# andreeaiana/manner

Hardware: AMD Instinct MI355X
Metric: candidate news encoded+scored/sec (higher is better)
Workload: dtype f16; 1 GPU; configs[1]: CR-Module late fusion, MIND-small shape (65238-news pool), bert-base-uncased architectu~; modules=1, parallelism=dp1 (impressions sharded, no collective)

## Files before the change

manner_amd/csrc/gemm.hip:

```cpp
#include <stdlib.h>

#include <type_traits>

#include "train_common.h"
#include "gemm_w4_asm.inc"
#include "gemm_w8_asm.inc"
#ifdef MANNER_P4_LAB
#include "gemm_p4_asm.inc"
#endif

namespace manner {
namespace {

constexpr int BM = 128, BN = 128, ROW_BYTES = 128, TILE_BYTES = 128 * ROW_BYTES;
constexpr int STAGE_BYTES = 2 * TILE_BYTES;

__device__ __forceinline__ float gelu_erf(float x) {
  return 0.5f * x * (1.0f + erff(x * 0.70710678118654752440f));
}

__device__ __forceinline__ float gelu_erf_fast(float x) {
  const float z = fabsf(x) * 0.70710678118654752440f;
  const float t = __builtin_amdgcn_rcpf(fmaf(0.3275911f, z, 1.0f));
  float p = fmaf(1.061405429f, t, -1.453152027f);
// ... 766 lines not shown
    } else {
      f32x4 bv[4], g4[4];
#pragma unroll
      for (int a = 0; a < 4; ++a) {
        bv[a] = *reinterpret_cast<const f32x4*>(bias + nbase + 16 * a + 4 * lq);
        g4[a] = *reinterpret_cast<const f32x4*>(dln.vec + nbase + 16 * a + 4 * lq);
      }
      char* rslab0 = slab;
      const int rrow0 = el >> 3, rsl = el & 7;
#pragma unroll
      for (int hb = 0; hb < (MBT + 3) / 4; ++hb) {
        const int nsb = MBT / 2 - 2 * hb >= 2 ? 2 : 1;
        const int nb4 = 2 * nsb;
        f32x4 rawres[2][4];
        float2 ms[4];
#pragma unroll
        for (int sb = 0; sb < nsb; ++sb)
#pragma unroll
          for (int q = 0; q < 4; ++q) {
            const int row = 8 * q + rrow0;
            const int m = min(mrow0 + 64 * hb + 32 * sb + row, M - 1);
            rawres[sb][q] = ABL == 3 ? f32x4{0.f, 0.f, 0.f, 0.f} : *reinterpret_cast<const f32x4*>(R + (size_t)m * N + nbase + 8 * (rsl ^ (row & 7)));
          }
#pragma unroll
        for (int b4 = 0; b4 < nb4; ++b4) ms[b4] = dln.mr[min(mrow0 + 16 * (4 * hb + b4) + l15, M - 1)];
        e16x4 res[4][4];
        if constexpr (!ONE_SLAB) {
#pragma unroll
          for (int sb = 0; sb < nsb; ++sb)
#pragma unroll
            for (int q = 0; q < 4; ++q) {
              const int row = 8 * q + rrow0;
              *reinterpret_cast<f32x4*>((sb ? rslab1 : rslab0) + row * 128 + (rsl << 4)) = rawres[sb][q];
            }
          __builtin_amdgcn_wave_barrier();
#pragma unroll
          for (int b4 = 0; b4 < nb4; ++b4) {
            const int row = 16 * (b4 & 1) + l15;
            const char* rs_ = (b4 >> 1) ? rslab1 : rslab0;
#pragma unroll
            for (int a = 0; a < 4; ++a) {
              const int c = (16 * a + 4 * lq) / 8;
              res[b4][a] = *reinterpret_cast<const e16x4*>(rs_ + row * 128 + ((c ^ (row & 7)) << 4) + 8 * (lq & 1));
            }
          }
          __builtin_amdgcn_wave_barrier();
        } else {
#pragma unroll
          for (int sb = 0; sb < nsb; ++sb) {
#pragma unroll
            for (int q = 0; q < 4; ++q) {
              const int row = 8 * q + rrow0;
              *reinterpret_cast<f32x4*>(rslab0 + row * 128 + (rsl << 4)) = rawres[sb][q];
            }
            __builtin_amdgcn_wave_barrier();
#pragma unroll
            for (int b2 = 0; b2 < 2; ++b2) {
              const int row = 16 * b2 + l15;
#pragma unroll
              for (int a = 0; a < 4; ++a) {
                const int c = (16 * a + 4 * lq) / 8;
                res[2 * sb + b2][a] = *reinterpret_cast<const e16x4*>(rslab0 + row * 128 + ((c ^ (row & 7)) << 4) + 8 * (lq & 1));
              }
            }
            __builtin_amdgcn_wave_barrier();
          }
        }
#pragma unroll
        for (int b4 = 0; b4 < nb4; ++b4) {
          const int bb = 4 * hb + b4;
          const float rs = ms[b4].y, nm = -ms[b4].x * ms[b4].y;
          float p1 = 0.f, p2 = 0.f;
#pragma unroll
          for (int a = 0; a < 4; ++a)
#pragma unroll
            for (int e = 0; e < 4; ++e) {
              const float r = fmaf((float)res[b4][a][e], rs, nm);
              const float x = fmaf(r, g4[a][e], acc[a][bb][e] + bv[a][e]);
              acc[a][bb][e] = x;
              p1 += x;
              p2 = fmaf(x, x, p2);
            }
          p1 += __shfl_xor(p1, 16, 64); p2 += __shfl_xor(p2, 16, 64);
          p1 += __shfl_xor(p1, 32, 64); p2 += __shfl_xor(p2, 32, 64);
          const int m = mrow0 + 16 * bb + l15;
          if (ABL == 4) asm volatile("" ::"v"(p1), "v"(p2));
          else if (ABL != 2 && lq == 0 && m < M)
            __hip_atomic_store(reinterpret_cast<unsigned long long*>(&dln.part[(size_t)(4 * nt + wn) * dln.part_stride + m]),
                               __builtin_bit_cast(unsigned long long, float2{p1, p2}), __ATOMIC_RELAXED, __HIP_MEMORY_SCOPE_AGENT);
        }
      }
    }
    if (ABL != 1) {
      const int row0 = el >> 3, sl = el & 7;
#pragma unroll
      for (int j = 0; j < MBT / 2; ++j) {
#pragma unroll
        for (int b2 = 0; b2 < 2; ++b2) {
          const int row = 16 * b2 + l15;
#pragma unroll
          for (int a = 0; a < 4; ++a) {
            const int c = (16 * a + 4 * lq) / 8;
            store4<TE>(reinterpret_cast<TE*>(slab + row * 128 + ((c ^ (row & 7)) << 4) + 8 * (lq & 1)),
                           acc[a][2 * j + b2][0], acc[a][2 * j + b2][1], acc[a][2 * j + b2][2], acc[a][2 * j + b2][3]);
          }
        }
        __builtin_amdgcn_wave_barrier();
#pragma unroll
        for (int q = 0; q < 4; ++q) {
          const int row = 8 * q + row0;
          const int c = sl ^ (row & 7);
          const int m = mrow0 + 32 * j + row;
          const f32x4 raw = *reinterpret_cast<const f32x4*>(slab + row * 128 + (sl << 4));
          if (m < M) *reinterpret_cast<f32x4*>(reinterpret_cast<TE*>(Y) + (size_t)m * N + nbase + 8 * c) = raw;
        }
        __builtin_amdgcn_wave_barrier();
      }
    }
    return;
  }
  int el = lane;
  asm volatile("" : "+v"(el));
  const int l15 = el & 15, lq = el >> 4, wn = ew & 3, wm = ew >> 2;
  const int nbase = nt * G_BN + wn * 64;
  const int row0 = el / CHUNKS, sl = el % CHUNKS;
  f32x4 bv[4];
#pragma unroll
  for (int a = 0; a < 4; ++a) bv[a] = *reinterpret_cast<const f32x4*>(bias + nbase + 16 * a + 4 * lq);
  constexpr bool NORM = EPI == EPI_NORM || EPI == EPI_NORM_GELU;
  constexpr bool SPLIT = EPI == EPI_BIAS_GELU_SPLIT3;
  const size_t ldy = SPLIT ? (size_t)3 * N : (size_t)N;
  f32x4 cv[NORM ? 4 : 1];
  float2 ms[NORM ? MBT : 1];
  const int mrow0 = mt * TM + wm * WROWS;
  if constexpr (NORM) {
#pragma unroll
    for (int a = 0; a < 4; ++a) cv[a] = *reinterpret_cast<const f32x4*>(dln.vec + nbase + 16 * a + 4 * lq);
#pragma unroll
    for (int bb = 0; bb < MBT; ++bb) ms[bb] = dln.mr[min(mrow0 + 16 * bb + l15, M - 1)];
  }
  constexpr int SLAB_ROWS = 4096 / OUT_ROW;
  constexpr int MB = SLAB_ROWS / 16;
  constexpr int SQ = SLAB_ROWS / ROWS_PER_INST;
#pragma unroll
  for (int j = 0; j < WROWS / SLAB_ROWS; ++j) {
#pragma unroll
    for (int b2 = 0; b2 < MB; ++b2) {
      const int row = 16 * b2 + l15;
#pragma unroll
      for (int a = 0; a < 4; ++a) {
        const int nl = 16 * a + 4 * lq;
        float v[4];
#pragma unroll
        for (int e = 0; e < 4; ++e) {
          if constexpr (NORM) v[e] = fmaf(ms[MB * j + b2].y, fmaf(-ms[MB * j + b2].x, cv[a][e], acc[a][MB * j + b2][e]), bv[a][e]);
          else v[e] = acc[a][MB * j + b2][e] + bv[a][e];
        }
        if (EPI == EPI_BIAS_GELU || EPI == EPI_NORM_GELU || SPLIT) {
#pragma unroll
          for (int e = 0; e < 4; ++e) v[e] = SPLIT ? gelu_erf_fast(v[e]) : sizeof(TOut) == 4 ? gelu_erf(v[e]) : gelu_poly(v[e]);
        }
        const int c = nl / OPC;
        const int off = row * OUT_ROW + ((c ^ (row & (CHUNKS - 1))) << 4) + (sizeof(TOut) == 2 ? 8 * (lq & 1) : 0);
        if constexpr (SPLIT) {
          typedef TOut o4 __attribute__((ext_vector_type(4)));
          o4 hv;
#pragma unroll
          for (int e = 0; e < 4; ++e) hv[e] = (TOut)v[e];
          asm volatile("" : "+v"(hv));
          *reinterpret_cast<o4*>(slab + off) = hv;
#pragma unroll
          for (int e = 0; e < 4; ++e) acc[a][MB * j + b2][e] = v[e] - (float)hv[e];
        } else {
          store4<TOut>(reinterpret_cast<TOut*>(slab + off), v[0], v[1], v[2], v[3]);
        }
      }
    }
    __builtin_amdgcn_wave_barrier();
    if constexpr (SPLIT) {
#pragma unroll
      for (int q = 0; q < SQ; ++q) {
        const int row = q * ROWS_PER_INST + row0;
        const int c = sl ^ (row & (CHUNKS - 1));
        const int m = mrow0 + SLAB_ROWS * j + row;
        const f32x4 raw = *reinterpret_cast<const f32x4*>(slab + row * OUT_ROW + (sl << 4));
        if (m < M) {
          TOut* dst = Y + (size_t)m * ldy + nbase + c * OPC;
          __builtin_nontemporal_store(raw, reinterpret_cast<f32x4*>(dst));
          __builtin_nontemporal_store(raw, reinterpret_cast<f32x4*>(dst + N));
        }
      }
      __builtin_amdgcn_wave_barrier();
#pragma unroll
      for (int b2 = 0; b2 < MB; ++b2) {
        const int row = 16 * b2 + l15;
#pragma unroll
        for (int a = 0; a < 4; ++a) {
          const int c = (16 * a + 4 * lq) / OPC;
          const int off = row * OUT_ROW + ((c ^ (row & (CHUNKS - 1))) << 4) + 8 * (lq & 1);
          store4<TOut>(reinterpret_cast<TOut*>(slab + off), acc[a][MB * j + b2][0], acc[a][MB * j + b2][1], acc[a][MB * j + b2][2],
                       acc[a][MB * j + b2][3]);
        }
      }
      __builtin_amdgcn_wave_barrier();
#pragma unroll
      for (int q = 0; q < SQ; ++q) {
        const int row = q * ROWS_PER_INST + row0;
        const int c = sl ^ (row & (CHUNKS - 1));
        const int m = mrow0 + SLAB_ROWS * j + row;
        const f32x4 raw = *reinterpret_cast<const f32x4*>(slab + row * OUT_ROW + (sl << 4));
        if (m < M) __builtin_nontemporal_store(raw, reinterpret_cast<f32x4*>(Y + (size_t)m * ldy + 2 * (size_t)N + nbase + c * OPC));
      }
      __builtin_amdgcn_wave_barrier();
      continue;
    }
    e16x4 res[EPI == EPI_BIAS_RES ? SQ : 1];
    f32x4 resf[EPI == EPI_BIAS_RES_F32 ? SQ : 1];
    if ((EPI == EPI_BIAS_RES || EPI == EPI_BIAS_RES_F32) && ABL != 1) {
#pragma unroll
      for (int q = 0; q < SQ; ++q) {
        const int row = q * ROWS_PER_INST + row0;
        const int m = min(mrow0 + SLAB_ROWS * j + row, M - 1);
        const size_t idx = (size_t)m * N + nbase + (sl ^ (row & (CHUNKS - 1))) * OPC;
        if (EPI == EPI_BIAS_RES) res[q] = *reinterpret_cast<const e16x4*>(R + idx);
        else resf[q] = *reinterpret_cast<const f32x4*>(reinterpret_cast<const float*>(R) + idx);
      }
    }
    f32x4 pre16v[EPI == EPI_GELU_GRAD16 ? SQ : 1];
    if constexpr (EPI == EPI_GELU_GRAD16) {
#pragma unroll
      for (int q = 0; q < SQ; ++q) {
        const int row = q * ROWS_PER_INST + row0;
        const int m = min(mrow0 + SLAB_ROWS * j + row, M - 1);
        pre16v[q] = *reinterpret_cast<const f32x4*>(static_cast<const TE*>(dln.pre16) + (size_t)m * N + nbase + (sl ^ (row & (CHUNKS - 1))) * OPC);
      }
    }
    f32x4 pre[EPI == EPI_GELU_GRAD ? SQ : 1][2];
    if constexpr (EPI == EPI_GELU_GRAD) {
#pragma unroll
      for (int q = 0; q < SQ; ++q) {
        const int row = q * ROWS_PER_INST + row0;
        const int m = min(mrow0 + SLAB_ROWS * j + row, M - 1);
        const f32x4* ip = reinterpret_cast<const f32x4*>(dln.aux32 + (size_t)m * N + nbase + (sl ^ (row & (CHUNKS - 1))) * OPC);
        pre[q][0] = ip[0];
        pre[q][1] = ip[1];
      }
    }
#pragma unroll
    for (int q = 0; q < SQ; ++q) {
      const int row = q * ROWS_PER_INST + row0;
      const int c = sl ^ (row & (CHUNKS - 1));
      const int m = mrow0 + SLAB_ROWS * j + row;
      f32x4 raw = *reinterpret_cast<const f32x4*>(slab + row * OUT_ROW + (sl << 4));
      if (ABL == 1) { asm volatile("" ::"v"(raw)); continue; }
      if constexpr (EPI == EPI_GELU_GRAD) {
        e16x8 d = __builtin_bit_cast(e16x8, raw);
#pragma unroll
        for (int e = 0; e < 8; ++e) d[e] = (TE)((float)d[e] * gelu_grad_fast(pre[q][e >> 2][e & 3]));
        raw = __builtin_bit_cast(f32x4, d);
      }
      if constexpr (EPI == EPI_GELU_GRAD16) {
        e16x8 d = __builtin_bit_cast(e16x8, raw);
        const e16x8 pv = __builtin_bit_cast(e16x8, pre16v[q]);
#pragma unroll
        for (int e = 0; e < 8; ++e) d[e] = (TE)((float)d[e] * gelu_grad_fast((float)pv[e]));
        raw = __builtin_bit_cast(f32x4, d);
      }
      if (EPI == EPI_BIAS_RES) {
#pragma unroll
        for (int e = 0; e < 4; ++e) raw[e] += (float)res[q][e];
      }
      if (EPI == EPI_BIAS_RES_F32) {
        if (dln.drop_thr != 0) {
          const uint64_t di = (uint64_t)(dln.drop_rowmap ? dln.drop_rowmap[min(m, M - 1)] : m) * N + (nbase + c * OPC);
#pragma unroll
          for (int e = 0; e < 4; ++e) raw[e] = drop_bits(dln.drop_seed, dln.drop_site, di + e) >= dln.drop_thr ? raw[e] * dln.drop_scale : 0.f;
        }
        raw += resf[q];
      }
      if (m < M) {
        f32x4* dst = reinterpret_cast<f32x4*>(reinterpret_cast<char*>(Y) + ((size_t)m * N + nbase + c * OPC) * sizeof(TOut));
        if (NORM && ABL != 5 && !dln.plain_stores) __builtin_nontemporal_store(raw, dst);
        else *dst = raw;
        if constexpr (EPI == EPI_BIAS_GELU_DUAL) {
          e16x4 gv;
#pragma unroll
          for (int e = 0; e < 4; ++e) gv[e] = (TE)gelu_erf_fast(raw[e]);
          *reinterpret_cast<e16x4*>(static_cast<TE*>(dln.aux16) + (size_t)m * N + nbase + c * OPC) = gv;
        }
        if constexpr (EPI == EPI_BIAS_GELU_DUAL16) {
          const e16x8 pv = __builtin_bit_cast(e16x8, raw);
          e16x8 gv;
#pragma unroll
          for (int e = 0; e < 8; ++e) gv[e] = (TE)gelu_erf_fast((float)pv[e]);
          *reinterpret_cast<e16x8*>(static_cast<TE*>(dln.aux16) + (size_t)m * N + nbase + c * OPC) = gv;
        }
      }
    }
    __builtin_amdgcn_wave_barrier();
  }
}


template <int TM>
__device__ __forceinline__ void nres_fan_in(const DlnAux& dln, int mt, int M, int n_tiles, int wave, int lane) {
  asm volatile("s_waitcnt vmcnt(0)" ::: "memory");
  __syncthreads();
  if (wave != 0) return;
  int old = 0;
  if (lane == 0) old = __hip_atomic_fetch_add(dln.fin_arrive + mt, 1, __ATOMIC_RELAXED, __HIP_MEMORY_SCOPE_AGENT);
  old = __builtin_amdgcn_readfirstlane(old);
  if (old != n_tiles - 1) return;
  constexpr int RPL = TM / 64;
  float2 v[RPL][16];
#pragma unroll
  for (int q = 0; q < RPL; ++q) {
    const int m = min(mt * TM + 64 * q + lane, M - 1);
#pragma unroll
    for (int g = 0; g < 16; ++g)
      v[q][g] = g < dln.fin_groups ? __builtin_bit_cast(float2, __hip_atomic_load(reinterpret_cast<const unsigned long long*>(&dln.part[(size_t)g * dln.part_stride + m]),
                                                                                  __ATOMIC_RELAXED, __HIP_MEMORY_SCOPE_AGENT))
                                   : float2{0.f, 0.f};
  }
#pragma unroll
  for (int q = 0; q < RPL; ++q) {
    const int m = mt * TM + 64 * q + lane;
    if (m < M) dln.fin_mr[m] = dln_row_stats(v[q], dln.fin_inv_h, dln.fin_eps);
  }
  if (lane == 0) __hip_atomic_store(dln.fin_arrive + mt, 0, __ATOMIC_RELAXED, __HIP_MEMORY_SCOPE_AGENT);
}

template <typename TE, typename TOut, int EPI, int ABL, int MBT>
__device__ __forceinline__ void gemm_tn_x16_body(
    char* lds, const TE* __restrict__ X, const TE* __restrict__ W, const float* __restrict__ bias,
    const TE* __restrict__ R, TOut* __restrict__ Y, int N, int K, int M, int n_tiles, const DlnAux& dln) {
  typedef TE TIn;
  typedef typename E16<TE>::v8 e16x8;
  constexpr int EPC = 8, BK = 64;
  constexpr int TM = 32 * MBT;
  constexpr int HB = MBT / 2;
  constexpr int WROWS = TM / 2;
  static_assert(MBT == 8 || MBT == 6, "row panels of 256 or 192 rows");
  constexpr int XB = 2 * G_OP_BYTES;

  const int G = gridDim.x, b = blockIdx.x;
  const int m_tiles = (MBT == 8 && dln.split_cus > 0) ? split_panels((M + TM - 1) / TM, n_tiles, dln.split_cus) : (M + TM - 1) / TM;
  const int valid_tiles = m_tiles * n_tiles;
  const int gsz = dln.col_group > 0 && dln.col_group < n_tiles ? dln.col_group : n_tiles;
  const int per_group = m_tiles * gsz;
  auto decode = [&](int tile, int& mt_, int& nt_) {
    const int g = tile / per_group;
    const int r = tile - g * per_group;
    const int width = min(gsz, n_tiles - g * gsz);
    mt_ = r / width;
    nt_ = g * gsz + (r - mt_ * width);
  };
  const TileWalk walk = tile_walk(G, b, valid_tiles, dln.xcd_ranges);
  int t = walk.first;
  if (t >= walk.end) return;
  if (dln.stagger > 0) {
    const int phase = (walk.first / n_tiles) & 3;
    for (int i = 0; i < phase * dln.stagger; ++i) __builtin_amdgcn_s_sleep(64);
  }

  const int tid = threadIdx.x, wave = __builtin_amdgcn_readfirstlane(tid >> 6), lane = tid & 63;
  const int kl15 = lane & 15, klq = lane >> 4;
  const int kwn = wave & 3, kwm = wave >> 2;

  const bool is_w = wave < 4;
  const int prow0 = is_w ? 64 * (wave & 3) : (TM / 4) * (wave & 3);
  const int ldst0 = (is_w ? 0 : XB) + prow0 * ROW_BYTES;
  const int lrow = lane >> 3;
  int voff[2];
#pragma unroll
  for (int par = 0; par < 2; ++par)
    voff[par] = lrow * K + (((lane & 7) ^ ((4 * par + (lane >> 4)) & 7)) * EPC);
  struct Src { const TIn* p; int lim; };
  auto tile_src = [&](int tile) -> Src {
    int mt_, nt_;
    decode(tile, mt_, nt_);
    if (is_w) return Src{W + (size_t)(nt_ * G_BN + prow0) * K, 64};
    if constexpr (MBT == 8) {
      return Src{X + (size_t)(mt_ * TM + prow0) * K, 64};
    } else {
      const int last = (int)dln.x_rows - 8;
      const int r0 = min(mt_ * TM + prow0, last);
      return Src{X + (size_t)r0 * K, min(last - r0, 64)};
    }
  };
  auto issue2 = [&](int buf, const Src& gsrc, int k0, int pair) {
    char* base = lds + buf * G_OP_BYTES + ldst0;
#pragma unroll
    for (int par = 0; par < 2; ++par) {
      const int i = 2 * pair + par;
      const int ro = MBT == 8 ? 8 * i : min(8 * i, gsrc.lim);
      if (ABL == 6 && !is_w)
        __builtin_amdgcn_global_load_lds(GLOBAL_PTR(gsrc.p + (size_t)ro * K + k0 + voff[par]), LDS_PTR(base + i * 1024), 16, 0, 2);
      else
        __builtin_amdgcn_global_load_lds(GLOBAL_PTR(gsrc.p + (size_t)ro * K + k0 + voff[par]),
                                         LDS_PTR(base + i * 1024), 16, 0, 0);
    }
  };

  const int swz = (kl15 >> 1) & 7;
  const int woff = (kwn * 64 + kl15) * ROW_BYTES;
  const int xoff = (kwm * WROWS + kl15) * ROW_BYTES;
  auto read_w = [&](const char* base, int s2, e16x8 (&wf)[4]) {
    const int coff = ((4 * s2 + klq) ^ swz) << 4;
#pragma unroll
    for (int a = 0; a < 4; ++a) wf[a] = *reinterpret_cast<const e16x8*>(base + woff + a * 16 * ROW_BYTES + coff);
  };
  auto read_x = [&](const char* base, int s2, int half, e16x8 (&xf)[HB]) {
    const int coff = ((4 * s2 + klq) ^ swz) << 4;
#pragma unroll
    for (int bb = 0; bb < HB; ++bb)
      xf[bb] = *reinterpret_cast<const e16x8*>(base + xoff + (HB * half + bb) * 16 * ROW_BYTES + coff);
  };

  f32x4 acc[4][MBT];
  auto mma16 = [&](const e16x8 (&wf)[4], const e16x8 (&xf)[HB], int half) {
#pragma unroll
    for (int bb = 0; bb < HB; ++bb)
#pragma unroll
      for (int a = 0; a < 4; ++a)
        acc[a][HB * half + bb] = E16<TE>::mfma16(wf[a], xf[bb], acc[a][HB * half + bb]);
  };

  e16x8 w0[4], w1[4], xa[HB], xb[HB];
  auto issue_all = [&](int buf, const Src& src, int k0) {
#pragma unroll
    for (int pair = 0; pair < 4; ++pair)
      if (MBT == 8 || pair < HB || is_w) issue2(buf, src, k0, pair);
  };
  auto kstep = [&](int cur, int xs, const Src& gsrc, int k1, int k2, const Src& gnext, bool has_next, auto mode_tag) {
    constexpr int MODE = decltype(mode_tag)::value;
    const char* wbase = lds + cur * G_OP_BYTES;
    const char* wnxt = lds + (cur ^ 1) * G_OP_BYTES;
    const int xs1 = xs == 2 ? 0 : xs + 1, xs2 = xs1 == 2 ? 0 : xs1 + 1;
    const char* xbase = lds + XB + xs * G_OP_BYTES;
    const char* xnxt = lds + XB + xs1 * G_OP_BYTES;
    if (ABL != 2 && !is_w) {
      if (MODE == 0) issue_all(xs2, gsrc, k2);
      else if (has_next) issue_all(xs2, gnext, MODE == 1 ? 0 : BK);
    }
    __builtin_amdgcn_sched_barrier(0);
    mma16(w0, xa, 0);
    __builtin_amdgcn_sched_barrier(0);
    read_x(xbase, 0, 1, xb);
    __builtin_amdgcn_sched_barrier(0);
    asm volatile("s_waitcnt lgkmcnt(0)" ::: "memory");
    mma16(w0, xb, 1);
    __builtin_amdgcn_sched_barrier(0);
    read_w(wbase, 1, w1);
    read_x(xbase, 1, 0, xa);
    __builtin_amdgcn_sched_barrier(0);
    asm volatile("s_waitcnt lgkmcnt(0)" ::: "memory");
    mma16(w1, xa, 0);
    __builtin_amdgcn_sched_barrier(0);
    read_x(xbase, 1, 1, xb);
    __builtin_amdgcn_sched_barrier(0);
    if (MODE <= 1) {
      if (is_w || (MODE == 1 && !has_next)) asm volatile("s_waitcnt vmcnt(0) lgkmcnt(0)" ::: "memory");
      else if constexpr (MBT == 8) asm volatile("s_waitcnt vmcnt(8) lgkmcnt(0)" ::: "memory");
      else asm volatile("s_waitcnt vmcnt(6) lgkmcnt(0)" ::: "memory");
    } else {
      asm volatile("s_waitcnt lgkmcnt(0)" ::: "memory");
    }
    __builtin_amdgcn_s_barrier();
    __builtin_amdgcn_sched_barrier(0);
    if (ABL != 2 && is_w) {
      if (MODE == 0) issue_all(cur, gsrc, k2);
      else if (MODE == 1 && has_next) issue_all(cur, gnext, 0);
    }
    __builtin_amdgcn_sched_barrier(0);
    mma16(w1, xb, 1);
    __builtin_amdgcn_sched_barrier(0);
    if (MODE <= 1) { read_w(wnxt, 0, w0); read_x(xnxt, 0, 0, xa); }
    __builtin_amdgcn_sched_barrier(0);
  };
  typedef std::integral_constant<int, 0> Mode0;
  typedef std::integral_constant<int, 1> Mode1;
  typedef std::integral_constant<int, 2> Mode2;

  const int nk = K / BK;

  Src gsrc = tile_src(t);
  issue_all(0, gsrc, 0);
  if (!is_w) issue_all(1, gsrc, BK);
  int buf = 0;
  int xs = 0;
  bool first = true;
  while (true) {
    int mt, nt;
    decode(t, mt, nt);
    const int tn = t + walk.stride;
    const bool has_next = tn < walk.end;
    const Src gnext = tile_src(has_next ? tn : t);
#pragma unroll
    for (int a = 0; a < 4; ++a)
#pragma unroll
      for (int bb = 0; bb < MBT; ++bb) acc[a][bb] = f32x4{0.f, 0.f, 0.f, 0.f};
    if (first) {
      if (is_w) asm volatile("s_waitcnt vmcnt(0)" ::: "memory");
      else if constexpr (MBT == 8) asm volatile("s_waitcnt vmcnt(8)" ::: "memory");
      else asm volatile("s_waitcnt vmcnt(6)" ::: "memory");
    } else if (ABL == 1) {
      asm volatile("s_waitcnt vmcnt(0)" ::: "memory");
    } else if (sizeof(TOut) == 2) {
      if constexpr (MBT == 8) asm volatile("s_waitcnt vmcnt(16)" ::: "memory");
      else asm volatile("s_waitcnt vmcnt(12)" ::: "memory");
    } else {
      asm volatile("s_waitcnt vmcnt(4)" ::: "memory");
    }
    first = false;
#ifdef MANNER_W8_STAMPS
    const uint64_t xst0 = __builtin_amdgcn_s_memtime();
#endif
    __builtin_amdgcn_s_barrier();
    read_w(lds + buf * G_OP_BYTES, 0, w0);
    read_x(lds + XB + xs * G_OP_BYTES, 0, 0, xa);
    if (ABL != 2 && is_w) issue_all(buf ^ 1, gsrc, BK);
    int kt = 0;
    for (; kt + 2 < nk; ++kt) {
      kstep((buf + kt) & 1, xs, gsrc, (kt + 1) * BK, (kt + 2) * BK, gnext, has_next, Mode0{});
      xs = xs == 2 ? 0 : xs + 1;
    }
    kstep((buf + kt) & 1, xs, gsrc, (kt + 1) * BK, 0, gnext, has_next, Mode1{});
    xs = xs == 2 ? 0 : xs + 1;
    ++kt;
    const int last = (buf + kt) & 1;
    kstep(last, xs, gsrc, 0, 0, gnext, has_next, Mode2{});
    const int xfree = xs;
    xs = xs == 2 ? 0 : xs + 1;
#ifdef MANNER_W8_STAMPS
    const uint64_t xst1 = __builtin_amdgcn_s_memtime();
#endif

    {
      int ew = wave;
      asm volatile("" : "+s"(ew));
      x16_epilogue<TE, TOut, EPI, ABL, MBT>(acc, lds + XB + xfree * G_OP_BYTES + ew * 4096, lds + last * G_OP_BYTES + ew * 4096, lane, ew, mt, nt, M, N,
                                             bias, R, Y, dln);
    }
    if constexpr (EPI == EPI_NRES && ABL == 0)
      if (dln.fin_mr) nres_fan_in<TM>(dln, mt, M, n_tiles, wave, lane);
#ifdef MANNER_W8_STAMPS
    if (dln.aux32) {
      const uint64_t xst2 = __builtin_amdgcn_s_memtime();
      uint64_t* dst = reinterpret_cast<uint64_t*>(const_cast<float*>(dln.aux32)) + ((size_t)blockIdx.x * 8 + wave) * 3;
      if (lane == 0) { dst[0] += xst1 - xst0; dst[1] += xst2 - xst1; dst[2] += 1; }
    }
#endif
    if (!has_next) break;
    t = tn;
    gsrc = gnext;
    buf = last ^ 1;
  }
}

template <typename TE, typename TOut, int EPI, int ABL = 0, bool PANELS = (ABL == 0)>
__global__ __launch_bounds__(512, 1) void gemm_tn_x16_kernel(
    const TE* __restrict__ X, const TE* __restrict__ W, const float* __restrict__ bias,
    const TE* __restrict__ R, TOut* __restrict__ Y, int N, int K, const int* __restrict__ m_total,
    int n_tiles, DlnAux dln) {
  __shared__ __attribute__((aligned(1024))) char lds[5 * G_OP_BYTES];
  if constexpr (EPI == EPI_BIAS) {
    X += (size_t)blockIdx.y * dln.batch_x;
    W += (size_t)blockIdx.y * dln.batch_w;
    Y += (size_t)blockIdx.y * dln.batch_y;
  }
  const int M = *m_total;
  if constexpr (PANELS) {
    if (panel_rows(M, n_tiles, (int)gridDim.x, dln.panel_mode) == 192) {
      gemm_tn_x16_body<TE, TOut, EPI, ABL, 6>(lds, X, W, bias, R, Y, N, K, M, n_tiles, dln);
      return;
    }
  }
  gemm_tn_x16_body<TE, TOut, EPI, ABL, 8>(lds, X, W, bias, R, Y, N, K, M, n_tiles, dln);
}

template <typename TE, typename TOut, int EPI, int ABL = 0>
__global__ __launch_bounds__(512, 1) void gemm_tn_w8_kernel(
    const TE* __restrict__ X, const TE* __restrict__ W, const float* __restrict__ bias,
    const TE* __restrict__ R, TOut* __restrict__ Y, int N, int K, const int* __restrict__ m_total,
    int n_tiles, DlnAux dln) {
  typedef typename E16<TE>::v8 e16x8;
  typedef float f32x16 __attribute__((ext_vector_type(16)));
  __shared__ __attribute__((aligned(1024))) char lds[5 * G_OP_BYTES];
  constexpr int BK = 64;
  if constexpr (EPI == EPI_BIAS) {
    X += (size_t)blockIdx.y * dln.batch_x;
    W += (size_t)blockIdx.y * dln.batch_w;
    Y += (size_t)blockIdx.y * dln.batch_y;
  }
  const int M = *m_total;
  const int G = gridDim.x, blk = blockIdx.x;
  const int m_tiles = (M + G_BM - 1) / G_BM;
  const int valid_tiles = m_tiles * n_tiles;
  const int gsz = dln.col_group > 0 && dln.col_group < n_tiles ? dln.col_group : n_tiles;
  const int per_group = m_tiles * gsz;
  auto decode = [&](int tile, int& mt_, int& nt_) {
    const int g = tile / per_group;
    const int r = tile - g * per_group;
    const int width = min(gsz, n_tiles - g * gsz);
    mt_ = r / width;
    nt_ = g * gsz + (r - mt_ * width);
  };
  const TileWalk walk = tile_walk(G, blk, valid_tiles, dln.xcd_ranges);
  int t = walk.first;
  if (t >= walk.end) return;

  const int tid = threadIdx.x, wave = __builtin_amdgcn_readfirstlane(tid >> 6), lane = tid & 63;
  const int wn = wave & 3, wm = wave >> 2;
  const int op = wave >> 2, qf = wave & 3;
  const int l15 = lane & 15, lq = lane >> 4, lrow = lane >> 3, lc = lane & 7;
  const uint32_t lds0 = (uint32_t)(uintptr_t)LDS_PTR(lds);
  if (lds0 & 0x1ffffu) __builtin_trap();
  const uint32_t swz = (l15 >> 1) & 7;
  uint32_t rw0 = lds0 + (64 * wn + l15) * ROW_BYTES + (((0 + lq) ^ swz) << 4);
  uint32_t rw1 = lds0 + (64 * wn + l15) * ROW_BYTES + (((4 + lq) ^ swz) << 4);
  uint32_t rx0 = lds0 + G_OP_BYTES + (128 * wm + l15) * ROW_BYTES + (((0 + lq) ^ swz) << 4);
  uint32_t rx1 = lds0 + G_OP_BYTES + (128 * wm + l15) * ROW_BYTES + (((4 + lq) ^ swz) << 4);
  const uint32_t wrow = lds0 + op * G_OP_BYTES + (64 * qf + lrow) * ROW_BYTES;
  uint32_t wa0 = 0x10000u + wrow + ((lc ^ (((lrow >> 1)) & 7)) << 4);
  uint32_t wa1 = 0x10000u + wrow + ((lc ^ ((4 + (lrow >> 1)) & 7)) << 4);
  const uint32_t d0 = (uint32_t)(((lc ^ ((lrow >> 1) & 7)) - lc) * 16), d1 = (uint32_t)(((lc ^ ((4 + (lrow >> 1)) & 7)) - lc) * 16);
  const uint32_t rowb = (uint32_t)K * 2u;
  const uint32_t lane_off = (uint32_t)lrow * rowb + (uint32_t)lc * 16u;
  uint32_t g = lane_off;
  const uint32_t c1 = 8 * rowb, c2 = 16 * rowb, c3 = 24 * rowb, c4 = 32 * rowb, c5 = 40 * rowb, c6 = 48 * rowb, c7 = 56 * rowb;
  auto tile_base = [&](int tile) -> const char* {
    int mt_, nt_;
    decode(tile, mt_, nt_);
    const TE* p_ = op == 0 ? W + (size_t)(nt_ * G_BN + 64 * qf) * K : X + (size_t)(mt_ * G_BM + 64 * qf) * K;
    return reinterpret_cast<const char*>(p_);
  };
  constexpr bool AGPR = EPI == EPI_NORM || EPI == EPI_NORM_GELU;
  e16x8 sa[8];
  {
    const char* cb = tile_base(t);
#pragma unroll
    for (int kt = 0; kt < 2; ++kt) {
      e16x8 v[8];
#pragma unroll
      for (int p = 0; p < 8; ++p) v[p] = *reinterpret_cast<const e16x8*>(cb + g + (uint32_t)p * 8u * rowb + kt * (BK * 2));
#pragma unroll
      for (int p = 0; p < 8; ++p) {
        if (AGPR && kt == 1) sa[p] = v[p];
        else *reinterpret_cast<e16x8*>(lds + (((p & 1) ? wa1 : wa0) - lds0 - (kt == 0 ? 0x10000u : 0u)) + p * 1024) = v[p];
      }
    }
    g += 256;
    __syncthreads();
  }
  const int nk = K / BK;
#ifdef MANNER_W8_SETPRIO
  if (wave >= 4) __builtin_amdgcn_s_setprio(1);
#endif
#ifdef MANNER_W8_STAMPS
  uint64_t stamp_k = 0, stamp_e = 0, stamp_n = 0;
#endif
  char* slab = lds + 4 * G_OP_BYTES + wave * 4096;
  while (true) {
    int mt, nt;
    decode(t, mt, nt);
    const int tn = t + walk.stride;
    const bool has_next = tn < walk.end;
    auto uniform = [](const char* p_) -> const char* {
      const uint64_t v = reinterpret_cast<uint64_t>(p_);
      const uint32_t lo = __builtin_amdgcn_readfirstlane((uint32_t)v), hi = __builtin_amdgcn_readfirstlane((uint32_t)(v >> 32));
      return reinterpret_cast<const char*>(((uint64_t)hi << 32) | lo);
    };
    const char* cbase = uniform(tile_base(t));
    const char* nbase = uniform(tile_base(has_next ? tn : t));
    int cnt = nk - 3;
    int m0_saved;
    (void)m0_saved;
    f32x16 o[8];
#ifdef MANNER_W8_STAMPS
    const uint64_t st0 = __builtin_amdgcn_s_memtime();
#endif
#define MANNER_W8_STATE [g] "+v"(g), [wa0] "+v"(wa0), [wa1] "+v"(wa1), [rw0] "+v"(rw0), [rw1] "+v"(rw1), [rx0] "+v"(rx0), [rx1] "+v"(rx1), [cnt] "+s"(cnt)
#define MANNER_W8_CONSTS                                                                                                                   \
  [base] "s"(cbase), [nbase] "s"(nbase), [rowb] "s"(rowb), [c1] "s"(c1), [c2] "s"(c2), [c3] "s"(c3), [c4] "s"(c4), [c5] "s"(c5),          \
      [c6] "s"(c6), [c7] "s"(c7)
#define MANNER_W8_RUN_TILE(MFMA_STR)                                                                                                       \
  asm volatile(MANNER_W8_TILE_ASM(MFMA_STR)                                                                                                \
               : MANNER_W8_ACC_OUTPUTS(o), MANNER_W8_STATE, [m0s] "=&s"(m0_saved)                                                          \
               : MANNER_W8_CONSTS, [d0] "v"(d0), [d1] "v"(d1)                                                                              \
               : MANNER_W8_CLOBBERS)
#define MANNER_W8_RUN_TILE_REGS(MFMA_STR)                                                                                                  \
  asm volatile(MANNER_W8_TILE_ASM_REGS(MFMA_STR)                                                                                           \
               : MANNER_W8_ACC_OUTPUTS(o), MANNER_W8_REGS_OPERANDS(sa), MANNER_W8_STATE                                                    \
               : MANNER_W8_CONSTS                                                                                                          \
               : MANNER_W8_CLOBBERS)
    if constexpr (AGPR) {
      if constexpr (E16<TE>::dtype == DT_BF16) {
        MANNER_W8_RUN_TILE_REGS("v_mfma_f32_16x16x32_bf16");
      } else {
        MANNER_W8_RUN_TILE_REGS("v_mfma_f32_16x16x32_f16");
      }
    } else {
      if constexpr (E16<TE>::dtype == DT_BF16) {
        MANNER_W8_RUN_TILE("v_mfma_f32_16x16x32_bf16");
      } else {
        MANNER_W8_RUN_TILE("v_mfma_f32_16x16x32_f16");
      }
    }
#undef MANNER_W8_RUN_TILE
#undef MANNER_W8_RUN_TILE_REGS
#undef MANNER_W8_STATE
#undef MANNER_W8_CONSTS
#ifdef MANNER_W8_STAMPS
    const uint64_t st1 = __builtin_amdgcn_s_memtime();
#endif
    {
      f32x4 acc[4][8];
#pragma unroll
      for (int a = 0; a < 4; ++a)
#pragma unroll
        for (int b = 0; b < 8; ++b) {
          const f32x16& s16 = o[2 * a + (b >> 2)];
          const int k4 = 4 * (b & 3);
          acc[a][b] = f32x4{s16[k4], s16[k4 + 1], s16[k4 + 2], s16[k4 + 3]};
        }
      int ew = wave;
      asm volatile("" : "+s"(ew));
      x16_epilogue<TE, TOut, EPI, ABL, 8, true>(acc, slab, slab, lane, ew, mt, nt, M, N, bias, R, Y, dln);
    }
    if constexpr (EPI == EPI_NRES && ABL == 0)
      if (dln.fin_mr) nres_fan_in<G_BM>(dln, mt, M, n_tiles, wave, lane);
#ifdef MANNER_W8_STAMPS
    {
      const uint64_t st2 = __builtin_amdgcn_s_memtime();
      stamp_k += st1 - st0; stamp_e += st2 - st1; stamp_n += 1;
    }
#endif
    if (!has_next) break;
    t = tn;
  }
#ifdef MANNER_W8_STAMPS
  if (lane == 0 && dln.aux32) {
    uint64_t* dst = reinterpret_cast<uint64_t*>(const_cast<float*>(dln.aux32)) + ((size_t)blk * 8 + wave) * 3;
    dst[0] = stamp_k; dst[1] = stamp_e; dst[2] = stamp_n;
  }
#endif
}

template <typename TE, typename TOut, int EPI>
__global__ __launch_bounds__(256, 1) void gemm_tn_w4_kernel(
    const TE* __restrict__ X, const TE* __restrict__ W, const float* __restrict__ bias,
    const TE* __restrict__ R, TOut* __restrict__ Y, int N, int K, const int* __restrict__ m_total,
    int n_tiles, DlnAux dln) {
  typedef typename E16<TE>::v8 e16x8;
  __shared__ __attribute__((aligned(1024))) char lds[5 * G_OP_BYTES];
  constexpr int BK = 64;
  const int M = *m_total;
  const int G = gridDim.x, blk = blockIdx.x;
  const int m_tiles = (M + G_BM - 1) / G_BM;
  const int valid_tiles = m_tiles * n_tiles;
  const int gsz = dln.col_group > 0 && dln.col_group < n_tiles ? dln.col_group : n_tiles;
  const int per_group = m_tiles * gsz;
  auto decode = [&](int tile, int& mt_, int& nt_) {
    const int g = tile / per_group;
    const int r = tile - g * per_group;
    const int width = min(gsz, n_tiles - g * gsz);
    mt_ = r / width;
    nt_ = g * gsz + (r - mt_ * width);
  };
  const TileWalk walk = tile_walk(G, blk, valid_tiles, dln.xcd_ranges);
  int t = walk.first;
  if (t >= walk.end) return;

  const int tid = threadIdx.x, wave = __builtin_amdgcn_readfirstlane(tid >> 6), lane = tid & 63;
  const int wn = wave & 1, wm = wave >> 1;
  const int op = wave >> 1, hf = wave & 1;
  const int l15 = lane & 15, lq = lane >> 4, lrow = lane >> 3, lc = lane & 7;
  const uint32_t lds0 = (uint32_t)(uintptr_t)LDS_PTR(lds);
  if (lds0 & 0x1ffffu) __builtin_trap();
  const uint32_t swz = (l15 >> 1) & 7;
  uint32_t rw0 = lds0 + (128 * wn + l15) * ROW_BYTES + (((0 + lq) ^ swz) << 4);
  uint32_t rw1 = lds0 + (128 * wn + l15) * ROW_BYTES + (((4 + lq) ^ swz) << 4);
  uint32_t rx0 = lds0 + G_OP_BYTES + (128 * wm + l15) * ROW_BYTES + (((0 + lq) ^ swz) << 4);
  uint32_t rx1 = lds0 + G_OP_BYTES + (128 * wm + l15) * ROW_BYTES + (((4 + lq) ^ swz) << 4);
  const uint32_t wrow = lds0 + op * G_OP_BYTES + (128 * hf + lrow) * ROW_BYTES;
  uint32_t wa0 = 0x10000u + wrow + ((lc ^ (((lrow >> 1)) & 7)) << 4);
  uint32_t wa1 = 0x10000u + wrow + ((lc ^ ((4 + (lrow >> 1)) & 7)) << 4);
  const uint32_t d0 = (uint32_t)(((lc ^ ((lrow >> 1) & 7)) - lc) * 16), d1 = (uint32_t)(((lc ^ ((4 + (lrow >> 1)) & 7)) - lc) * 16);
  const uint32_t rowb = (uint32_t)K * 2u;
  const uint32_t lane_off = (uint32_t)lrow * rowb + (uint32_t)lc * 16u;
  uint32_t g = lane_off;
  const uint32_t c1 = 8 * rowb, c2 = 16 * rowb, c3 = 24 * rowb, c4 = 32 * rowb, c5 = 40 * rowb, c6 = 48 * rowb, c7 = 56 * rowb, c8 = 64 * rowb,
                 c9 = 72 * rowb, c10 = 80 * rowb, c11 = 88 * rowb, c12 = 96 * rowb, c13 = 104 * rowb, c14 = 112 * rowb, c15 = 120 * rowb;
  auto tile_base = [&](int tile) -> const char* {
    int mt_, nt_;
    decode(tile, mt_, nt_);
    const TE* p_ = op == 0 ? W + (size_t)(nt_ * G_BN + 128 * hf) * K : X + (size_t)(mt_ * G_BM + 128 * hf) * K;
    return reinterpret_cast<const char*>(p_);
  };
  {
    const char* cb = tile_base(t);
#pragma unroll
    for (int kt = 0; kt < 2; ++kt) {
      e16x8 v[16];
#pragma unroll
      for (int p = 0; p < 16; ++p) v[p] = *reinterpret_cast<const e16x8*>(cb + g + (uint32_t)p * 8u * rowb + kt * (BK * 2));
#pragma unroll
      for (int p = 0; p < 16; ++p)
        *reinterpret_cast<e16x8*>(lds + (((p & 1) ? wa1 : wa0) - lds0 - (kt == 0 ? 0x10000u : 0u)) + p * 1024) = v[p];
    }
    g += 256;
    __syncthreads();
  }
  const int nk = K / BK;
  char* slab = lds + 4 * G_OP_BYTES + wave * 8192;
  while (true) {
    int mt, nt;
    decode(t, mt, nt);
    const int tn = t + walk.stride;
    const bool has_next = tn < walk.end;
    auto uniform = [](const char* p_) -> const char* {
      const uint64_t v = reinterpret_cast<uint64_t>(p_);
      const uint32_t lo = __builtin_amdgcn_readfirstlane((uint32_t)v), hi = __builtin_amdgcn_readfirstlane((uint32_t)(v >> 32));
      return reinterpret_cast<const char*>(((uint64_t)hi << 32) | lo);
    };
    const char* cbase = uniform(tile_base(t));
    const char* nbase = uniform(tile_base(has_next ? tn : t));
    int cnt = nk - 3;
    int m0_saved;
#define MANNER_W4_RUN_TILE(MFMA_STR)                                                                                                       \
  asm volatile(MANNER_W4_TILE_ASM(MFMA_STR)                                                                                                \
               : [g] "+v"(g), [wa0] "+v"(wa0), [wa1] "+v"(wa1), [rw0] "+v"(rw0), [rw1] "+v"(rw1), [rx0] "+v"(rx0), [rx1] "+v"(rx1),        \
                 [cnt] "+s"(cnt), [m0s] "=&s"(m0_saved)                                                                                    \
               : [base] "s"(cbase), [nbase] "s"(nbase), [rowb] "s"(rowb), [d0] "v"(d0), [d1] "v"(d1), [c1] "s"(c1), [c2] "s"(c2),         \
                 [c3] "s"(c3), [c4] "s"(c4), [c5] "s"(c5), [c6] "s"(c6), [c7] "s"(c7), [c8] "s"(c8), [c9] "s"(c9), [c10] "s"(c10),         \
                 [c11] "s"(c11), [c12] "s"(c12), [c13] "s"(c13), [c14] "s"(c14), [c15] "s"(c15)                                            \
               : MANNER_W4_CLOBBERS)
    if constexpr (E16<TE>::dtype == DT_BF16) {
      MANNER_W4_RUN_TILE("v_mfma_f32_16x16x32_bf16");
    } else {
      MANNER_W4_RUN_TILE("v_mfma_f32_16x16x32_f16");
    }
#undef MANNER_W4_RUN_TILE
    {
      f32x4 acc[4][8];
      MANNER_W4_READ_HALF0(acc)
      int ew = 4 * wm + 2 * wn;
      asm volatile("" : "+s"(ew));
      x16_epilogue<TE, TOut, EPI, 0, 8>(acc, slab, slab + 4096, lane, ew, mt, nt, M, N, bias, R, Y, dln);
    }
    {
      f32x4 acc[4][8];
      MANNER_W4_READ_HALF1(acc)
      int ew = 4 * wm + 2 * wn + 1;
      asm volatile("" : "+s"(ew));
      x16_epilogue<TE, TOut, EPI, 0, 8>(acc, slab, slab + 4096, lane, ew, mt, nt, M, N, bias, R, Y, dln);
    }
    if (!has_next) break;
    t = tn;
  }
}

#ifdef MANNER_P4_LAB
template <typename TE, typename TOut, int EPI, int ABL = 0>
__global__ __launch_bounds__(256, 2) void gemm_tn_p4_kernel(
    const TE* __restrict__ X, const TE* __restrict__ W, const float* __restrict__ bias,
    const TE* __restrict__ R, TOut* __restrict__ Y, int N, int K, const int* __restrict__ m_total,
    int n_tiles, DlnAux dln) {
  typedef typename E16<TE>::v8 e16x8;
  constexpr int P4_W = 0, P4_X = 16384, P4_SLAB = 49152;
  __shared__ __attribute__((aligned(1024))) char lds[65536];
  constexpr int BK = 64;
  const int M = *m_total;
  const int G = gridDim.x, blk = blockIdx.x;
  const int m_tiles = (M + G_BM - 1) / G_BM;
  const int n_half = 2 * n_tiles;
  const int valid_tiles = m_tiles * n_half;
  const int gsz = dln.col_group > 0 && dln.col_group < n_tiles ? 2 * dln.col_group : n_half;
  const int per_group = m_tiles * gsz;
  auto decode = [&](int tile, int& mt_, int& nh_) {
    const int g_ = tile / per_group;
    const int r = tile - g_ * per_group;
    const int width = min(gsz, n_half - g_ * gsz);
    mt_ = r / width;
    nh_ = g_ * gsz + (r - mt_ * width);
  };
  const TileWalk walk = tile_walk(G, blk, valid_tiles, dln.xcd_ranges);
  int t = walk.first;
  if (t >= walk.end) return;

  const int tid = threadIdx.x, wave = __builtin_amdgcn_readfirstlane(tid >> 6), lane = tid & 63;
  const int wn = wave & 1, wm = wave >> 1;
  const int l15 = lane & 15, lq = lane >> 4, lrow = lane >> 3, lc = lane & 7;
  const uint32_t lds0 = (uint32_t)(uintptr_t)LDS_PTR(lds);
  const uint32_t swz = (l15 >> 1) & 7;
  const uint32_t rw0 = lds0 + P4_W + (64 * wn + l15) * ROW_BYTES + (((0 + lq) ^ swz) << 4);
  const uint32_t rw1 = lds0 + P4_W + (64 * wn + l15) * ROW_BYTES + (((4 + lq) ^ swz) << 4);
  const uint32_t rx0 = lds0 + P4_X + (128 * wm + l15) * ROW_BYTES + (((0 + lq) ^ swz) << 4);
  const uint32_t rx1 = lds0 + P4_X + (128 * wm + l15) * ROW_BYTES + (((4 + lq) ^ swz) << 4);
  const uint32_t sw0 = (lc ^ ((lrow >> 1) & 7)) << 4, sw1 = (lc ^ ((4 + (lrow >> 1)) & 7)) << 4;
  const uint32_t ww0 = lds0 + P4_W + (32 * wave + lrow) * ROW_BYTES + sw0, ww1 = lds0 + P4_W + (32 * wave + lrow) * ROW_BYTES + sw1;
  const uint32_t xw0 = lds0 + P4_X + (64 * wave + lrow) * ROW_BYTES + sw0, xw1 = lds0 + P4_X + (64 * wave + lrow) * ROW_BYTES + sw1;
  const uint32_t rowb = (uint32_t)K * 2u;
  const uint32_t lane_off = (uint32_t)lrow * rowb + (uint32_t)lc * 16u;
  uint32_t g = lane_off;
  const uint32_t c1 = 8 * rowb, c2 = 16 * rowb, c3 = 24 * rowb, c4 = 32 * rowb, c5 = 40 * rowb, c6 = 48 * rowb, c7 = 56 * rowb;
  auto uniform = [](const char* p_) -> const char* {
    const uint64_t v = reinterpret_cast<uint64_t>(p_);
    const uint32_t lo = __builtin_amdgcn_readfirstlane((uint32_t)v), hi = __builtin_amdgcn_readfirstlane((uint32_t)(v >> 32));
    return reinterpret_cast<const char*>(((uint64_t)hi << 32) | lo);
  };
  auto w_share = [&](int tile) -> const char* {
    int mt_, nh_;
    decode(tile, mt_, nh_);
    return reinterpret_cast<const char*>(W + (size_t)(nh_ * 128 + 32 * wave) * K);
  };
  auto x_share = [&](int tile) -> const char* {
    int mt_, nh_;
    decode(tile, mt_, nh_);
    return reinterpret_cast<const char*>(X + (size_t)(mt_ * G_BM + 64 * wave) * K);
  };
  if ((dln.stagger & 0xff) > 0) {
    const uint32_t hw = __builtin_amdgcn_s_getreg((4 << 0) | (0 << 6) | (31 << 11));
    const int mode = dln.stagger >> 8;
    const bool second = mode == 0 ? (hw >> 16) & 1 : mode == 1 ? hw & 1 : mode == 2 ? (blk >> 3) & 1 : (blk >> 3) >= (G >> 4);
    if (second)
      for (int i = 0; i < (dln.stagger & 0xff); ++i) __builtin_amdgcn_s_sleep(127);
  }
  {
    const char* wb = w_share(t);
    const char* xb = x_share(t);
    e16x8 v[12];
#pragma unroll
    for (int p = 0; p < 4; ++p) v[p] = *reinterpret_cast<const e16x8*>(wb + g + (uint32_t)p * 8u * rowb);
#pragma unroll
    for (int p = 0; p < 8; ++p) v[4 + p] = *reinterpret_cast<const e16x8*>(xb + g + (uint32_t)p * 8u * rowb);
#pragma unroll
    for (int p = 0; p < 4; ++p) *reinterpret_cast<e16x8*>(lds + (((p & 1) ? ww1 : ww0) - lds0) + p * 1024) = v[p];
#pragma unroll
    for (int p = 0; p < 8; ++p) *reinterpret_cast<e16x8*>(lds + (((p & 1) ? xw1 : xw0) - lds0) + p * 1024) = v[4 + p];
    g += 128;
    __syncthreads();
  }
  const int nk = K / BK;
  char* slab = lds + P4_SLAB + wave * 4096;
  while (true) {
    int mt, nh;
    decode(t, mt, nh);
    const int tn = t + walk.stride;
    const bool has_next = tn < walk.end;
    const char* cbw = uniform(w_share(t));
    const char* cbx = uniform(x_share(t));
    const char* nbw = uniform(w_share(has_next ? tn : t));
    const char* nbx = uniform(x_share(has_next ? tn : t));
    int cnt = nk - 3;
    f32x16 o[8];
#define MANNER_P4_RUN_TILE(MFMA_STR)                                                                                                       \
  asm volatile(MANNER_P4_TILE_ASM(MFMA_STR)                                                                                                \
               : MANNER_P4_ACC_OUTPUTS(o), [g] "+v"(g), [cnt] "+s"(cnt)                                                                    \
               : [ww0] "v"(ww0), [ww1] "v"(ww1), [xw0] "v"(xw0), [xw1] "v"(xw1), [rw0] "v"(rw0), [rw1] "v"(rw1), [rx0] "v"(rx0),            \
                 [rx1] "v"(rx1), [basew] "s"(cbw), [basex] "s"(cbx), [nbasew] "s"(nbw), [nbasex] "s"(nbx), [rowb] "s"(rowb), [c1] "s"(c1), \
                 [c2] "s"(c2), [c3] "s"(c3), [c4] "s"(c4), [c5] "s"(c5), [c6] "s"(c6), [c7] "s"(c7)                                        \
               : MANNER_P4_CLOBBERS)
    if constexpr (E16<TE>::dtype == DT_BF16) {
      MANNER_P4_RUN_TILE("v_mfma_f32_16x16x32_bf16");
    } else {
      MANNER_P4_RUN_TILE("v_mfma_f32_16x16x32_f16");
    }
#undef MANNER_P4_RUN_TILE
    {
      f32x4 acc[4][8];
#pragma unroll
      for (int a = 0; a < 4; ++a)
#pragma unroll
        for (int b = 0; b < 8; ++b) {
          const f32x16& s16 = o[2 * a + (b >> 2)];
          const int k4 = 4 * (b & 3);
          acc[a][b] = f32x4{s16[k4], s16[k4 + 1], s16[k4 + 2], s16[k4 + 3]};
        }
      int ew = 4 * wm + 2 * (nh & 1) + wn;
      asm volatile("" : "+s"(ew));
      x16_epilogue<TE, TOut, EPI, ABL, 8, true>(acc, slab, slab, lane, ew, mt, nh >> 1, M, N, bias, R, Y, dln);
    }
    if (!has_next) break;
    t = tn;
  }
}
#endif

static int x16_grid(int64_t m_bound, int n_tiles, DlnAux& aux, dim3& g) {
  const int64_t tiles = ((m_bound + 191) / 192) * n_tiles;
  if (tiles <= 0 || tiles > 0x7fffffff) return fail(MANNER_HIP_E_INVALID, "gemm grid %lld out of range", (long long)tiles);
  const int n_cus = device_cus();
  g = dim3((unsigned)(tiles < n_cus ? tiles : n_cus));
  const char* e = getenv("MANNER_HIP_GEMM_PANEL");
  aux.panel_mode = e ? (atoi(e) == 256 ? 1 : atoi(e) == 192 ? 2 : 0) : 0;
  aux.x_rows = m_bound;
  return MANNER_HIP_OK;
}

static int pick_asm(int64_t m_est, int n_tiles, int K, const DlnAux& aux) {
  const char* e = getenv("MANNER_HIP_GEMM_ASM");
  const int req = e ? atoi(e) : 8;
  if (req != 8 && req != 4) return 0;
  if (aux.stagger != 0 || aux.split_cus > 0 || K % 64 || K < 192 || aux.panel_mode == 2) return 0;
  return panel_rows((int)m_est, n_tiles, device_cus(), aux.panel_mode) == 256 ? req : 0;
}

static int pick_col_group(int64_t m_est, int N, int K, int cus) {
  const int n_tiles = N / G_BN;
  const double w_bytes = 2.0 * N * K, x_bytes = 2.0 * (double)m_est * K, l2_keep = 2.5 * 1048576.0;
  const int64_t rounds = ((m_est + G_BM - 1) / G_BM * n_tiles + cus - 1) / cus;
  if (w_bytes <= l2_keep) return 0;
  const int groups = (int)((w_bytes + l2_keep - 1) / l2_keep);
  return (groups - 1) * x_bytes < 8.0 * (double)(rounds - 1) * w_bytes ? (n_tiles + groups - 1) / groups : 0;
}

static void set_tile_order(DlnAux& aux, int64_t m_est, int N, int K) {
  const char* cg_env = getenv("MANNER_HIP_COL_GROUP");
  const char* xr_env = getenv("MANNER_HIP_XCD_RANGES");
  aux.xcd_ranges = xr_env ? (atoi(xr_env) != 0) : 1;
  aux.col_group = cg_env ? atoi(cg_env) : aux.xcd_ranges ? pick_col_group(m_est, N, K, device_cus()) : 0;
}

template <typename TE, typename TOut>
int launch_x16(Epilogue epi, const void* X, const void* W, const float* bias, const void* R, void* Y,
               int64_t m_bound, int N, int K, const int* m_total, hipStream_t stream) {
  const int n_tiles = N / G_BN;
  DlnAux aux0{};
  set_tile_order(aux0, m_bound, N, K);
  if (epi == EPI_BIAS_GELU_SPLIT3 && !getenv("MANNER_HIP_XCD_RANGES")) aux0.xcd_ranges = aux0.col_group = 0;
// ... 415 lines not shown
```

Measured before the change: 44520 candidates/s.

## Add specialized W8 residual-layernorm epilogue with software-pipelined residual loads

```diff
diff --git a/manner_amd/csrc/gemm.hip b/manner_amd/csrc/gemm.hip
--- a/manner_amd/csrc/gemm.hip
+++ b/manner_amd/csrc/gemm.hip
@@ -1092,6 +1092,132 @@
 }
 
 
+__device__ __forceinline__ float xsum16(float p) {
+  float a = p, b = p;
+  asm volatile("s_nop 1\n\tv_permlane16_swap_b32 %0, %1" : "+v"(a), "+v"(b));
+  return a + b;
+}
+__device__ __forceinline__ float xsum32(float p) {
+  float a = p, b = p;
+  asm volatile("s_nop 1\n\tv_permlane32_swap_b32 %0, %1" : "+v"(a), "+v"(b));
+  return a + b;
+}
+
+template <typename TE, int ABL>
+__device__ __forceinline__ void w8_nres_epilogue(f32x4 (&acc)[4][8], char* slab, int lane, int ew, int mt, int nt, int M, int N,
+                                                 const float* __restrict__ bias, const TE* __restrict__ R, TE* __restrict__ Y, const DlnAux& dln) {
+  typedef typename E16<TE>::v4 e16x4;
+  int el = lane;
+  asm volatile("" : "+v"(el));
+  const int l15 = el & 15, lq = el >> 4, wn = ew & 3, wm = ew >> 2;
+  const int nbase = nt * G_BN + wn * 64;
+  const int mrow0 = mt * G_BM + wm * 128;
+  const int rrow0 = el >> 3, rsl = el & 7;
+  f32x4 bv[4], g4[4];
+#pragma unroll
+  for (int a = 0; a < 4; ++a) {
+    bv[a] = *reinterpret_cast<const f32x4*>(bias + nbase + 16 * a + 4 * lq);
+    g4[a] = *reinterpret_cast<const f32x4*>(dln.vec + nbase + 16 * a + 4 * lq);
+  }
+  auto load_sb = [&](int hb, int sb, f32x4 (&raw)[4]) {
+#pragma unroll
+    for (int q = 0; q < 4; ++q) {
+      const int row = 8 * q + rrow0;
+      const int m = min(mrow0 + 64 * hb + 32 * sb + row, M - 1);
+      raw[q] = ABL == 3 ? f32x4{0.f, 0.f, 0.f, 0.f} : *reinterpret_cast<const f32x4*>(R + (size_t)m * N + nbase + 8 * (rsl ^ (row & 7)));
+    }
+  };
+  auto load_ms = [&](int hb, float2 (&ms)[4]) {
+#pragma unroll
+    for (int b4 = 0; b4 < 4; ++b4) ms[b4] = dln.mr[min(mrow0 + 16 * (4 * hb + b4) + l15, M - 1)];
+  };
+  auto transpose = [&](const f32x4 (&raw)[2][4], e16x4 (&res)[4][4]) {
+#pragma unroll
+    for (int sb = 0; sb < 2; ++sb) {
+#pragma unroll
+      for (int q = 0; q < 4; ++q) {
+        const int row = 8 * q + rrow0;
+        *reinterpret_cast<f32x4*>(slab + row * 128 + (rsl << 4)) = raw[sb][q];
+      }
+      __builtin_amdgcn_wave_barrier();
+#pragma unroll
+      for (int b2 = 0; b2 < 2; ++b2) {
+        const int row = 16 * b2 + l15;
+#pragma unroll
+        for (int a = 0; a < 4; ++a) {
+          const int c = (16 * a + 4 * lq) / 8;
+          res[2 * sb + b2][a] = *reinterpret_cast<const e16x4*>(slab + row * 128 + ((c ^ (row & 7)) << 4) + 8 * (lq & 1));
+        }
+      }
+      __builtin_amdgcn_wave_barrier();
+    }
+  };
+  auto arith = [&](int hb, const e16x4 (&res)[4][4], const float2 (&ms)[4]) {
+#pragma unroll
+    for (int b4 = 0; b4 < 4; ++b4) {
+      const int bb = 4 * hb + b4;
+      const float rs = ms[b4].y, nm = -ms[b4].x * ms[b4].y;
+      float p1 = 0.f, p2 = 0.f;
+#pragma unroll
+      for (int a = 0; a < 4; ++a)
+#pragma unroll
+        for (int e = 0; e < 4; ++e) {
+          const float r = fmaf((float)res[b4][a][e], rs, nm);
+          const float x = fmaf(r, g4[a][e], acc[a][bb][e] + bv[a][e]);
+          acc[a][bb][e] = x;
+          p1 += x;
+          p2 = fmaf(x, x, p2);
+        }
+      p1 = xsum16(p1); p2 = xsum16(p2);
+      p1 = xsum32(p1); p2 = xsum32(p2);
+      const int m = mrow0 + 16 * bb + l15;
+      if (ABL == 4) asm volatile("" ::"v"(p1), "v"(p2));
+      else if (ABL != 2 && lq == 0 && m < M)
+        __hip_atomic_store(reinterpret_cast<unsigned long long*>(&dln.part[(size_t)(4 * nt + wn) * dln.part_stride + m]),
+                           __builtin_bit_cast(unsigned long long, float2{p1, p2}), __ATOMIC_RELAXED, __HIP_MEMORY_SCOPE_AGENT);
+    }
+  };
+  auto store_half = [&](int hb) {
+    const int row0 = el >> 3, sl = el & 7;
+#pragma unroll
+    for (int jj = 0; jj < 2; ++jj) {
+      const int j = 2 * hb + jj;
+#pragma unroll
+      for (int b2 = 0; b2 < 2; ++b2) {
+        const int row = 16 * b2 + l15;
+#pragma unroll
+        for (int a = 0; a < 4; ++a) {
+          const int c = (16 * a + 4 * lq) / 8;
+          store4<TE>(reinterpret_cast<TE*>(slab + row * 128 + ((c ^ (row & 7)) << 4) + 8 * (lq & 1)),
+                     acc[a][2 * j + b2][0], acc[a][2 * j + b2][1], acc[a][2 * j + b2][2], acc[a][2 * j + b2][3]);
+        }
+      }
+      __builtin_amdgcn_wave_barrier();
+#pragma unroll
+      for (int q = 0; q < 4; ++q) {
+        const int row = 8 * q + row0;
+        const int c = sl ^ (row & 7);
+        const int m = mrow0 + 32 * j + row;
+        const f32x4 raw = *reinterpret_cast<const f32x4*>(slab + row * 128 + (sl << 4));
+        if (m < M) *reinterpret_cast<f32x4*>(Y + (size_t)m * N + nbase + 8 * c) = raw;
+      }
+      __builtin_amdgcn_wave_barrier();
+    }
+  };
+  f32x4 raw[2][4];
+  float2 ms0[4], ms1[4];
+  e16x4 res[4][4];
+  load_sb(0, 0, raw[0]); load_sb(0, 1, raw[1]); load_ms(0, ms0);
+  transpose(raw, res);
+  load_sb(1, 0, raw[0]);
+  arith(0, res, ms0);
+  load_sb(1, 1, raw[1]); load_ms(1, ms1);
+  store_half(0);
+  transpose(raw, res);
+  arith(1, res, ms1);
+  store_half(1);
+}
+
 template <int TM>
 __device__ __forceinline__ void nres_fan_in(const DlnAux& dln, int mt, int M, int n_tiles, int wave, int lane) {
   asm volatile("s_waitcnt vmcnt(0)" ::: "memory");
@@ -1112,6 +1238,7 @@
                                                                                   __ATOMIC_RELAXED, __HIP_MEMORY_SCOPE_AGENT))
                                    : float2{0.f, 0.f};
   }
+  __builtin_amdgcn_s_waitcnt(0xF70);
 #pragma unroll
   for (int q = 0; q < RPL; ++q) {
     const int m = mt * TM + 64 * q + lane;
@@ -1516,7 +1643,10 @@
         }
       int ew = wave;
       asm volatile("" : "+s"(ew));
-      x16_epilogue<TE, TOut, EPI, ABL, 8, true>(acc, slab, slab, lane, ew, mt, nt, M, N, bias, R, Y, dln);
+      if constexpr (EPI == EPI_NRES && ABL != 1)
+        w8_nres_epilogue<TE, ABL>(acc, slab, lane, ew, mt, nt, M, N, bias, R, reinterpret_cast<TE*>(Y), dln);
+      else
+        x16_epilogue<TE, TOut, EPI, ABL, 8, true>(acc, slab, slab, lane, ew, mt, nt, M, N, bias, R, Y, dln);
     }
     if constexpr (EPI == EPI_NRES && ABL == 0)
       if (dln.fin_mr) nres_fan_in<G_BM>(dln, mt, M, n_tiles, wave, lane);
```

New measurement: 44640 candidates/s (median of 6 runs). Within noise of the previous version (+0.3%).
